# DINT-NSDI24/DINT

Measured on AMD Instinct MI355X. Metric: Mtxn/s + p50/p99 batch latency, TATP, higher is better.
Workload: dtype u64

## Files before the change

### dint_amd/csrc/dint_kv.h

```cpp
#pragma once
#include <cstdlib>
#include <utility>
#include <vector>

#include "dint_kernels.h"
#include "dint_kv_core.h"
#include "state_block.h"
#include "state_image.h"
#include "state_route.h"

#define DINT_KV_MAX_TABLES 5
#define DINT_KV_CTL_BYTES (64 + 24 * KV_NLISTS)
#define DINT_KV_TRACE_WORDS ((size_t)DINT_KV_PMAX * 16 + 16 * 8192)
#define DINT_KV_LOAD_OP 0xF0u

struct kv_dev {
  kv_tab tab[DINT_KV_MAX_TABLES];
  dint_mod mod[DINT_KV_MAX_TABLES];
  dint_mod lockmod[DINT_KV_MAX_TABLES];
  uint32_t gk_base[DINT_KV_MAX_TABLES];
  uint32_t n_tables;
  uint32_t shard_index, shard_count;
  uint32_t same_key;
  uint32_t pass_ins[DINT_KV_MAX_TABLES];
};

struct dint_kv_knobs {
  uint32_t coarse_load = 512;
  uint32_t cap = 0;
  uint32_t lcap = 1024;
  uint32_t cap_mult = 64;
  uint32_t rpt = 0;
  uint32_t no_bm = 0;
  uint32_t hot_min = 0;
  uint32_t no_split = 0;
  uint32_t split_min = 65;
  uint32_t split_target = 384;
  uint32_t one_big_kernel = 0;
  uint32_t workers = 96;
  uint32_t part_first = 0;
  uint32_t sb_split_min = 65;
  uint32_t sb_npmax = 128;
  uint32_t sb_workers = 130;
  uint32_t sb_late_grid = 32;
  uint32_t residency = 0;
  uint32_t no_fuse = 0;
  uint32_t no_ahead = 0;
  uint32_t late_grid = 8;
  uint32_t exp_no_late = 0;
  uint32_t late_fat = 0;
  uint32_t late_big = 0;
};

struct dint_kv {
  uint32_t workload = 0;
  uint32_t n_tables = 0;
  uint32_t val_size = 0;
  int force_rounds = 0;
  uint64_t hash_size[DINT_KV_MAX_TABLES] = {0, 0, 0, 0, 0};
  kv_dev h{};
  kv_dev *d_dev = nullptr;
  uint8_t *d_ctl = nullptr;
  uint64_t *d_trace = nullptr;
  size_t entry_bytes[DINT_KV_MAX_TABLES] = {0, 0, 0, 0, 0};
  dint_kv_knobs knobs;
};

static inline uint32_t dint_kv_cap_mult() {
  const char *v = getenv("DINT_KV_CAP_MULT");
  const unsigned long m = v && *v ? strtoul(v, nullptr, 10) : 64ul;
  return (uint32_t)(m < 2 ? 2 : m > 256 ? 256 : m);
}
static inline uint32_t dint_kv_hash_sizes(uint32_t workload, uint64_t n_rows, uint64_t hs[DINT_KV_MAX_TABLES], uint32_t *val_size) {
  uint32_t n_tables;
  for (uint32_t t = 0; t < DINT_KV_MAX_TABLES; t++) hs[t] = 0;
  if (workload == DINT_WL_STORE) {
    const uint64_t n = n_rows ? n_rows : 2000000ull;
    n_tables = 1;
    *val_size = 40;
    hs[0] = n * 18 / 4;
  } else if (workload == DINT_WL_TATP) {
    const uint64_t n = n_rows ? n_rows : 7000000ull;
    n_tables = 5;
    *val_size = 40;
    hs[0] = hs[1] = n * 3 / 2 / 4;
    hs[2] = hs[3] = n * 15 / 4 / 4;
    hs[4] = n * 45 / 8 / 4;
  } else {
    const uint64_t n = n_rows ? n_rows : 24000000ull;
    n_tables = 2;
    *val_size = 8;
    hs[0] = hs[1] = n * 3 / 2 / 4;
  }
  for (uint32_t t = 0; t < n_tables; t++)
    if (hs[t] == 0) hs[t] = 1;
  return n_tables;
}
int dint_kv_create(dint_kv *kv, uint32_t workload, uint64_t n_rows, dint_shard shard, uint32_t pool_entries = 0,
                   uint32_t flags = 0);
void dint_kv_destroy(dint_kv *kv);
std::vector<std::pair<void *, size_t>> dint_kv_regions(dint_kv *kv);
int64_t dint_kv_dump_rows(dint_kv *kv, uint32_t table, uint64_t *keys, uint32_t *vers, uint8_t *vals, uint64_t cap);
int64_t dint_kv_read_locks(dint_kv *kv, uint32_t table, uint32_t *a, uint32_t *b, uint64_t cap);
struct dint_kv_ahead {
  const void *d_req;
  void *d_rep;
  uint32_t n;
  dint_view view;
};
bool dint_kv_ahead_ok(const dint_kv &kv, int load_mode);
bool dint_kv_one_launch(const dint_kv &kv, int load_mode);
void dint_launch_kv(const void *d_req, void *d_rep, uint32_t n, const dint_kv &kv, dint_log log, dint_scratch s,
                    int load_mode, hipStream_t st, hipEvent_t *ev, const dint_view &view = dint_flat_view(),
                    bool part_done = false, const dint_kv_ahead *next = nullptr);
#define DINT_KV_MULTI_MAX 4u
struct dint_kv_pass {
  const void *d_req;
  void *d_rep;
  uint32_t n;
  const dint_kv *kv;
  dint_log log;
  dint_scratch s;
  dint_view view;
};
void dint_launch_kv_multi(const dint_kv_pass *p, uint32_t n_eng, hipStream_t st, bool part_done = false, const dint_kv_pass *next = nullptr);
bool dint_kv_multi_ahead_ok(const dint_kv &kv);
void dint_launch_home_kv(const void *d_req, uint32_t n, const dint_kv &kv, uint8_t *d_home, hipStream_t st);
struct dint_kv_fmt {
  uint32_t msg, type, table, key, val, ver, val_size;
};
dint_kv_fmt dint_kv_format(uint32_t workload);

struct dint_state_scratch {
  unsigned long long *words;
  uint32_t *blk_cnt;
  uint64_t *blk_off;
  uint32_t nb;
  unsigned long long *digest_part;
};
#define DINT_STATE_DIGEST_GRID 2048u
#define DINT_STATE_WORDS 48u
#define DINT_STATE_DIGEST_AT 16u
uint32_t dint_state_blocks(const dint_kv &kv);
void dint_launch_state_digest(const dint_kv &kv, dint_state_scratch s, hipStream_t st);
void dint_launch_state_diff_count(const dint_kv &a, const dint_kv &b, dint_state_scratch s, hipStream_t st);
void dint_launch_state_diff_write(const dint_kv &a, const dint_kv &b, dint_state_scratch s, void *d_records, uint64_t cap, hipStream_t st);
void dint_launch_state_repair_check(const dint_kv &kv, const void *d_records, uint64_t n, dint_state_scratch s, hipStream_t st);
#define DINT_STATE_HOME_AT 14u
void dint_launch_state_home_check(const dint_kv &kv, const void *d_records, uint64_t n, dint_state_scratch s, hipStream_t st);
void dint_launch_state_repair(const dint_kv &kv, const void *d_records, uint64_t n, uint32_t pend_set, dint_dev_stats *stats,
                              dint_state_scratch s, hipStream_t st);

#define DINT_STATE_STATS_GRID 2048u
#define DINT_STATE_STATS_WORDS 80u
struct dint_stats_scratch {
  unsigned long long *part;
  unsigned long long *out;
};
void dint_launch_state_stats(const dint_kv &kv, dint_stats_scratch s, hipStream_t st);

#define DINT_STATE_VERIFY_GRID 2048u
#define DINT_STATE_VERIFY_WORDS 32u
#define DINT_STATE_VERIFY_PARTS (2u * DINT_STATE_VERIFY_GRID + 1u)
struct dint_verify_scratch {
  uint32_t *owner;
  uint64_t owner_n;
  unsigned long long *part;
  unsigned long long *out;
  uint32_t *leaked;
  uint32_t *blk_cnt;
  uint64_t *blk_off;
  uint64_t blk_n;
  unsigned long long *heads;
};
int dint_verify_alloc(const dint_kv &kv, dint_verify_scratch &s, uint32_t flags);
void dint_verify_free(dint_verify_scratch &s);
void dint_launch_state_verify(const dint_kv &kv, dint_verify_scratch s, uint32_t flags, hipStream_t st, hipEvent_t *ev = nullptr);
int dint_verify_collect(const dint_kv &kv, dint_verify_scratch s, uint32_t flags, hipStream_t st, struct dint_table_verify *out,
                        uint64_t *reclaimed);

struct dint_tables_view;
int dint_view_kv(const dint_tables_view *v, const void *out, uint32_t cap_tables, dint_kv *kv);

// ... 156 lines not shown
```

### dint_amd/csrc/k_kv.hip

```cpp
#include "k_kv_dev.h"

dint_kv_fmt dint_kv_format(uint32_t workload) {
  switch (workload) {
    case DINT_WL_STORE: return {53, 0, 0xFFFFFFFFu, 1, 9, 49, 40};
    case DINT_WL_TATP: return {55, 1, 2, 3, 11, 51, 40};
    default: return {23, 1, 2, 3, 11, 19, 8};
  }
}


static inline uint32_t kv_pick_coarse(uint32_t n, uint32_t load) {
  uint64_t c = ((uint64_t)n + load - 1) / load;
  if (c < 1) c = 1;
  if (c > DINT_KV_CMAX) c = DINT_KV_CMAX;
  return (uint32_t)c;
}
static uint32_t kv_env(const char *name, uint32_t dflt) {
  const char *v = getenv(name);
  return v && *v ? (uint32_t)strtoul(v, nullptr, 10) : dflt;
}
static dint_kv_knobs kv_read_knobs() {
  dint_kv_knobs k;
  k.coarse_load = std::min(8192u, std::max(64u, kv_env("DINT_KV_COARSE_LOAD", KVB_T)));
  k.cap = kv_env("DINT_KV_CAP", 0);
  k.lcap = std::min(KVR_LCAP, kv_env("DINT_KV_LCAP", KVR_LCAP));
  k.cap_mult = dint_kv_cap_mult();
  k.rpt = kv_env("DINT_KV_RPT", 0);
  k.no_bm = kv_env("DINT_KV_NO_BM", 0);
  k.hot_min = kv_env("DINT_KV_HOT_MIN", 0);
  k.no_split = kv_env("DINT_KV_NO_SPLIT", 0);
  k.split_min = std::max(65u, kv_env("DINT_KV_SPLIT_MIN", 65u));
  k.split_target = std::min(448u, std::max(8u, kv_env("DINT_KV_SPLIT_TARGET", 384u)));
  k.one_big_kernel = kv_env("DINT_KV_ONE_BIG_KERNEL", 0);
  k.no_ahead = kv_env("DINT_KV_NO_AHEAD", 0);
  k.no_fuse = kv_env("DINT_KV_NO_FUSE", 0);
  k.sb_split_min = kv_env("DINT_KV_SB_SPLIT_MIN", 65u);
  k.sb_late_grid = std::max(1u, std::min(KVB_GRID, kv_env("DINT_KV_SB_LATE_GRID", 32u)));
  k.sb_npmax = std::max(2u, std::min(KSB_NPMAX, kv_env("DINT_KV_SB_NPMAX", 128u)));
  k.sb_workers = kv_env("DINT_KV_SB_WORKERS", k.sb_npmax + 2u);
  if (k.sb_workers) k.sb_workers = std::max(k.sb_workers, k.sb_npmax + 2u);
  k.workers = std::min(1024u, std::max(KVR_NPMAX + 2u, kv_env("DINT_KV_WORKERS", KVW_GRID)));
  k.part_first = kv_env("DINT_KV_PART_FIRST", 0) & 1u;
  k.late_grid = std::min(KVB_GRID, std::max(1u, kv_env("DINT_KV_LATE_GRID", 8u)));
  k.late_big = kv_env("DINT_KV_LATE_BIG", 0);
  k.exp_no_late = kv_env("DINT_EXP_NO_LATE", 0);
  k.late_fat = kv_env("DINT_KV_LATE_FAT", 0);
  return k;
}

static inline bool kv_uses_hot(const dint_kv &kv, int load_mode) {
  return kv.workload != DINT_WL_SMALLBANK && !(kv.force_rounds & 3) && !load_mode && !kv.knobs.no_split;
}
bool dint_kv_one_launch(const dint_kv &kv, int load_mode) {
  return kv_uses_hot(kv, load_mode) && !kv.knobs.one_big_kernel && !kv.knobs.no_fuse;
}
bool dint_kv_ahead_ok(const dint_kv &kv, int load_mode) {
  if (kv.workload == DINT_WL_SMALLBANK) return !load_mode && !kv.knobs.no_ahead && !kv.knobs.no_fuse;
  return kv_uses_hot(kv, load_mode) && !kv.knobs.one_big_kernel && !kv.knobs.no_ahead;
}

static void kv_fill_pass(kv_pass_args &A, const void *d_req, void *d_rep, uint32_t n, const dint_kv &kv, dint_log log,
                         const dint_scratch &s, int load_mode, const dint_view &view, uint32_t tile) {
  const dint_kv_knobs &K = kv.knobs;
  const uint32_t C = kv_pick_coarse(n, K.coarse_load);
  const uint32_t mean = (n + C - 1) / C;
  uint32_t cap = K.cap_mult * mean + 64;
  cap = std::min(cap, (uint32_t)(s.kbins_slots / C));
  cap = std::max(1u, K.cap ? std::min(cap, K.cap) : cap);
  A.req = (const uint8_t *)d_req; A.rep = (uint8_t *)d_rep; A.n = n;
  A.n_tiles = (n + tile - 1) / tile;
  A.kv = kv.d_dev; A.log = log; A.cut = kv_make_cut(C, n); A.cap = cap;
  A.lcap = K.lcap;
  const uint64_t pn = s.kvs.pass_no;
  A.pno = (uint32_t)(pn & 1u);
  A.bin_cnt = s.kvs.bin_cnt[pn & 1]; A.kbins = s.kvs.kbins[pn & 1]; A.ovl = s.kvs.ovl[pn & 1];
  A.big = s.kvs.ctl[pn % 3]; A.big_z = s.kvs.ctl[(pn + 2) % 3];
  A.blk_pub = s.kvs.pub[pn % 3]; A.blk_pub_z = s.kvs.pub[(pn + 2) % 3];
  A.bigrdy = s.kvs.bigrdy;
  A.ovf = s.ovf; A.ovf2 = s.ovf2; A.stats = s.stats;
  A.bigq = s.bigq;
  A.hotpub = s.hotpub;
  A.lateq = s.lateq;
  A.seq = s.pass_seq ? s.pass_seq : 1u;
  A.inv_n = n > 1 ? (uint32_t)((1ull << 32) / n) : 0xFFFFFFFFu;
  A.load_mode = load_mode;
  A.force_flags = kv.force_rounds | (K.no_bm ? 4 : 0) | (int)(K.hot_min << 8);
  A.split_min = kv_uses_hot(kv, load_mode) ? K.split_min : 0xFFFFFFFFu;
  A.split_target = K.split_target;
  A.np_max = KVR_NPMAX;
  A.sb_pieces = 0;
  A.sbx = s.kvs.sbx;
  if (kv.workload == DINT_WL_SMALLBANK && K.sb_split_min && s.kvs.sbx && !(kv.force_rounds & 3) && !load_mode && !K.no_split) {
    A.split_min = std::max(8u, K.sb_split_min);
    A.np_max = K.sb_npmax;
    A.sb_pieces = 1;
  }
  A.has_log = kv.workload != DINT_WL_STORE;
  A.trace = kv.d_trace;
  A.V = view;
}

extern template int kv_piece_residency<DINT_WL_STORE>(int);
extern template int kv_piece_residency<DINT_WL_TATP>(int);
extern template int kv_piece_residency<DINT_WL_SMALLBANK>(int);
extern template void launch_kv_passes<DINT_WL_STORE>(kv_multi_args &, uint32_t, uint32_t, hipStream_t, hipEvent_t *, const dint_kv_knobs &, bool, const kv_multi_args *, uint32_t);
extern template void launch_kv_passes<DINT_WL_TATP>(kv_multi_args &, uint32_t, uint32_t, hipStream_t, hipEvent_t *, const dint_kv_knobs &, bool, const kv_multi_args *, uint32_t);
extern template void launch_kv_passes<DINT_WL_SMALLBANK>(kv_multi_args &, uint32_t, uint32_t, hipStream_t, hipEvent_t *, const dint_kv_knobs &, bool, const kv_multi_args *, uint32_t);

static inline uint32_t kv_pick_rpt(uint32_t n_total, const dint_kv_knobs &K) {
  if (K.rpt == 1 || K.rpt == 2 || K.rpt == 4) return K.rpt;
  return n_total >= 1024u * 1024u ? 4u : n_total >= 256u * 1024u ? 2u : 1u;
}
static inline uint32_t kv_pick_rpt_ahead(uint32_t n, const dint_kv_knobs &K) {
  if (K.rpt == 4 || (K.rpt == 0 && n >= 256u * 1024u)) return 4u;
  return 2u;
}

static void launch_kv_dispatch(uint32_t workload, kv_multi_args &M, uint32_t n_eng, uint32_t rpt, hipStream_t st, hipEvent_t *ev,
                               const dint_kv_knobs &K, bool part_done = false, const kv_multi_args *next = nullptr, uint32_t next_rpt = 0) {
  switch (workload) {
    case DINT_WL_STORE: launch_kv_passes<DINT_WL_STORE>(M, n_eng, rpt, st, ev, K, part_done, next, next_rpt); break;
    case DINT_WL_TATP: launch_kv_passes<DINT_WL_TATP>(M, n_eng, rpt, st, ev, K, part_done, next, next_rpt); break;
    default: launch_kv_passes<DINT_WL_SMALLBANK>(M, n_eng, rpt, st, ev, K, part_done, next, next_rpt); break;
  }
}

void dint_launch_kv(const void *d_req, void *d_rep, uint32_t n, const dint_kv &kv, dint_log log, dint_scratch s,
                    int load_mode, hipStream_t st, hipEvent_t *ev, const dint_view &view, bool part_done, const dint_kv_ahead *next) {
  if (n == 0) return;
  kv_multi_args M;
  memset(&M, 0, sizeof M);
  const uint32_t rpt = kv_pick_rpt(n, kv.knobs), rpt_a = kv_pick_rpt_ahead(n, kv.knobs);
  kv_fill_pass(M.e[0], d_req, d_rep, n, kv, log, s, load_mode, view, part_done ? KVB_T * rpt_a : KV_TB * rpt);
  kv_multi_args N;
  uint32_t next_rpt = 0;
  if (next && next->n && dint_kv_ahead_ok(kv, load_mode)) {
    dint_scratch sn = s;
    sn.kvs.pass_no = s.kvs.pass_no + 1;
    sn.pass_seq = s.pass_seq + 1 >= 0x3FFFFFFFu ? 1u : s.pass_seq + 1;
    next_rpt = kv_pick_rpt_ahead(next->n, kv.knobs);
    memset(&N, 0, sizeof N);
    kv_fill_pass(N.e[0], next->d_req, next->d_rep, next->n, kv, log, sn, load_mode, next->view, KVB_T * next_rpt);
  } else {
    next = nullptr;
  }
  launch_kv_dispatch(kv.workload, M, 1, rpt, st, ev, kv.knobs, part_done, next ? &N : nullptr, next_rpt);
}

void dint_launch_kv_multi(const dint_kv_pass *p, uint32_t n_eng, hipStream_t st, bool part_done, const dint_kv_pass *next) {
  if (n_eng == 0) return;
  kv_multi_args M, N;
  memset(&M, 0, sizeof M);
  uint32_t n_total = 0;
  for (uint32_t k = 0; k < n_eng; k++) n_total += p[k].n;
  const uint32_t rpt = kv_pick_rpt(n_total, p[0].kv->knobs);
  for (uint32_t k = 0; k < n_eng; k++) kv_fill_pass(M.e[k], p[k].d_req, p[k].d_rep, p[k].n, *p[k].kv, p[k].log, p[k].s, 0, p[k].view, KV_TB * rpt);
  uint32_t next_rpt = 0;
  if (next) {
    uint32_t nmax = 0;
    for (uint32_t k = 0; k < n_eng; k++) nmax = std::max(nmax, next[k].n);
    next_rpt = kv_pick_rpt_ahead(nmax, p[0].kv->knobs);
    memset(&N, 0, sizeof N);
    for (uint32_t k = 0; k < n_eng; k++) {
      dint_scratch sn = next[k].s;
      sn.kvs.pass_no = p[k].s.kvs.pass_no + 1;
      sn.pass_seq = p[k].s.pass_seq + 1 >= 0x3FFFFFFFu ? 1u : p[k].s.pass_seq + 1;
      kv_fill_pass(N.e[k], next[k].d_req, next[k].d_rep, next[k].n, *next[k].kv, next[k].log, sn, 0, next[k].view, KVB_T * next_rpt);
    }
  }
  launch_kv_dispatch(p[0].kv->workload, M, n_eng, rpt, st, nullptr, p[0].kv->knobs, part_done, next ? &N : nullptr, next_rpt);
}
bool dint_kv_multi_ahead_ok(const dint_kv &kv) { return dint_kv_ahead_ok(kv, 0) && !kv.knobs.no_fuse; }

__global__ void __launch_bounds__(256)
k_home_kv(const uint8_t *__restrict__ req, uint32_t n, const kv_dev *__restrict__ kv, dint_kv_fmt f,
          uint8_t *__restrict__ home) {
  const uint32_t i = blockIdx.x * 256u + threadIdx.x;
  if (i >= n) return;
  const uint8_t *m = req + (size_t)i * f.msg;
  const uint32_t table = f.table == 0xFFFFFFFFu ? 0 : m[f.table];
  if (table >= kv->n_tables) { home[i] = 0xFF; return; }
  const uint64_t g = dint_fastmod(dint_hash_key(ld_u64(m + f.key)), kv->mod[table]);
  home[i] = (uint8_t)(g % (kv->shard_count ? kv->shard_count : 1));
}
void dint_launch_home_kv(const void *d_req, uint32_t n, const dint_kv &kv, uint8_t *d_home, hipStream_t st) {
  if (n == 0) return;
  hipLaunchKernelGGL(k_home_kv, dim3((n + 255) / 256), dim3(256), 0, st, (const uint8_t *)d_req, n, kv.d_dev,
                     dint_kv_format(kv.workload), d_home);
}

int dint_kv_create(dint_kv *kv, uint32_t workload, uint64_t n_rows, dint_shard shard, uint32_t pool_entries,
                   uint32_t flags) {
  *kv = dint_kv();
  kv->workload = workload;
  kv->h.same_key = (workload == DINT_WL_TATP && (flags & DINT_FLAG_LOCK_SAME_KEY)) ? 1 : 0;
  uint64_t hs[DINT_KV_MAX_TABLES] = {0, 0, 0, 0, 0};
  kv->n_tables = dint_kv_hash_sizes(workload, n_rows, hs, &kv->val_size);
  const uint32_t stride = kv->val_size == 40 ? 256u : 128u;
  const uint32_t count = shard.count ? shard.count : 1;
  kv->h.n_tables = kv->n_tables;
  kv->h.shard_index = shard.index;
  kv->h.shard_count = count;
  for (uint32_t t = 0; t < DINT_KV_MAX_TABLES; t++) kv->h.pass_ins[t] = 0xFFFFFFFFu;
  if (hipMalloc((void **)&kv->d_ctl, DINT_KV_CTL_BYTES * DINT_KV_MAX_TABLES) != hipSuccess) return DINT_ENOMEM;
  hipMemset(kv->d_ctl, 0, DINT_KV_CTL_BYTES * DINT_KV_MAX_TABLES);
  uint64_t gk = 0;
  for (uint32_t t = 0; t < kv->n_tables; t++) {
    if (hs[t] == 0) hs[t] = 1;
    kv->hash_size[t] = hs[t];
    kv_tab &tb = kv->h.tab[t];
    tb.n_local = (hs[t] + count - 1) / count;
    const uint64_t pool = pool_entries ? pool_entries : tb.n_local / 4 + 4096;
    if (pool > 0xFFFFFFF0ull || gk + tb.n_local > 0xFFFFFFF0ull) return DINT_EINVAL;
    tb.pool_cap = (uint32_t)pool;
    tb.stride = stride;
    tb.val_size = kv->val_size;
    kv->entry_bytes[t] = (size_t)(tb.n_local + tb.pool_cap) * stride;
    if (hipMalloc((void **)&tb.entries, kv->entry_bytes[t]) != hipSuccess) return DINT_ENOMEM;
    if (hipMemset(tb.entries, 0, kv->entry_bytes[t]) != hipSuccess) return DINT_EHIP;
    if (hipMalloc((void **)&tb.pool_next, (size_t)tb.pool_cap * 4) != hipSuccess) return DINT_ENOMEM;
    hipMemset(tb.pool_next, 0, (size_t)tb.pool_cap * 4);
    uint8_t *ctl = kv->d_ctl + DINT_KV_CTL_BYTES * t;
    tb.pool_top = (uint32_t *)ctl;
    tb.free_head = (unsigned long long *)(ctl + 64);
    tb.pend_head = (unsigned long long *)(ctl + 64 + 8 * KV_NLISTS);
// ... 162 lines not shown
```

### dint_amd/csrc/k_kv_dev.h

```cpp
#pragma once
#include <algorithm>
#include <cstddef>
#include <cstdlib>
#include <cstring>
#include <utility>
#include <vector>

#include "../../include/dint_abi.h"
#include "dint_kv.h"
#define KVB_SORT_INLINE
#include "dint_bins.h"

template <int WL> struct Fmt;
template <> struct Fmt<DINT_WL_STORE> {
  static constexpr uint32_t MSG = 53, TYPE = 0, KEY = 1, VAL = 9, VER = 49, VS = 40;
  static constexpr bool HAS_TABLE = false;
  static constexpr uint32_t TABLE = 0;
};
template <> struct Fmt<DINT_WL_TATP> {
  static constexpr uint32_t MSG = 55, TYPE = 1, KEY = 3, VAL = 11, VER = 51, VS = 40;
  static constexpr bool HAS_TABLE = true;
  static constexpr uint32_t TABLE = 2;
};
template <> struct Fmt<DINT_WL_SMALLBANK> {
  static constexpr uint32_t MSG = 23, TYPE = 1, KEY = 3, VAL = 11, VER = 19, VS = 8;
  static constexpr bool HAS_TABLE = true;
  static constexpr uint32_t TABLE = 2;
};

template <int WL>
__device__ static inline uint32_t kv_class(uint32_t type, int load_mode) {
  if (load_mode && type == DINT_KV_LOAD_OP) return 1;
  if (WL == DINT_WL_STORE) return type <= 2 ? 1 : 0;
  if (WL == DINT_WL_TATP) {
    switch (type) {
      case 0: case 1: case 2: case 12: case 13: case 18: case 19: case 22: case 23: return 1;
      case 14: case 24: return 2;
      default: return 0;
    }
  }
  return (type <= 5 || type == 17) ? 1 : (type == 6 ? 2 : 0);
}

__device__ static inline uint32_t kv_pay(uint32_t type, uint32_t q, uint32_t kh) {
  return (type == DINT_KV_LOAD_OP ? 31u : type) | (q << 5) | (kh << 7);
}
__device__ static inline uint32_t pay_type(uint32_t p) { const uint32_t t = p & 31u; return t == 31u ? DINT_KV_LOAD_OP : t; }
__device__ static inline uint32_t pay_q(uint32_t p) { return (p >> 5) & 3u; }
__device__ static inline uint32_t pay_kh(uint32_t p) { return (p >> 7) & 511u; }
__device__ static inline uint32_t kv_table_of(const kv_dev *kv, uint32_t gk) {
  uint32_t t = 0;
  for (uint32_t k = 1; k < kv->n_tables; k++) t += gk >= kv->gk_base[k];
  return t;
}

__device__ static inline uint64_t ld_u64(const uint8_t *p) { uint64_t v; __builtin_memcpy(&v, p, 8); return v; }
__device__ static inline uint32_t ld_u32(const uint8_t *p) { uint32_t v; __builtin_memcpy(&v, p, 4); return v; }
__device__ static inline void st_u32(uint8_t *p, uint32_t v) { __builtin_memcpy(p, &v, 4); }

struct kv_dev_mem {
  __device__ static inline uint32_t fetch_add(uint32_t *p, uint32_t v) { return atomicAdd(p, v); }
  __device__ static inline uint32_t load32(uint32_t *p) { return atomicAdd(p, 0u); }
  __device__ static inline void store32(uint32_t *p, uint32_t v) { atomicExch(p, v); }
  __device__ static inline unsigned long long load64(unsigned long long *p) { return atomicAdd(p, 0ull); }
  __device__ static inline bool cas64(unsigned long long *p, unsigned long long exp, unsigned long long des) {
    return atomicCAS(p, exp, des) == exp;
  }
};

__device__ static inline void kv_dev_pend_set(kv_dev &Skv, uint32_t pno) {
  if (threadIdx.x < DINT_KV_MAX_TABLES && (pno & 1u)) Skv.tab[threadIdx.x].pend_head += KV_NLISTS;
}
#define KV_CTL_INS 32u
static_assert(KV_CTL_INS + DINT_KV_MAX_TABLES <= DINT_KV_CTL_WORDS && KV_CTL_INS * 4 >= 128, "a set of control words is DINT_KV_CTL_WORDS; the counts on a line of their own");
__device__ static inline uint32_t kv_dev_word(const kv_dev *kv, const uint32_t *ctl, uint32_t w) {
  constexpr uint32_t at = (uint32_t)(offsetof(kv_dev, pass_ins) / 4);
  return w >= at && w < at + DINT_KV_MAX_TABLES ? ctl[KV_CTL_INS + w - at] : ((const uint32_t *)kv)[w];
}
__device__ static inline void kv_st_agent(uint64_t *p, uint64_t v) { __hip_atomic_store((unsigned long long *)p, (unsigned long long)v, __ATOMIC_RELAXED, __HIP_MEMORY_SCOPE_AGENT); }
__device__ static inline uint64_t kv_ld_agent(const uint64_t *p) { return __hip_atomic_load((const unsigned long long *)p, __ATOMIC_RELAXED, __HIP_MEMORY_SCOPE_AGENT); }
__device__ static inline void kv_st_agent(uint4 *p, const uint4 &v) {
  kv_st_agent((uint64_t *)p, ((uint64_t)v.y << 32) | v.x);
  kv_st_agent((uint64_t *)p + 1, ((uint64_t)v.w << 32) | v.z);
}
__device__ static inline uint4 kv_ld_agent(const uint4 *p) {
  const uint64_t a = kv_ld_agent((const uint64_t *)p), b = kv_ld_agent((const uint64_t *)p + 1);
  return make_uint4((uint32_t)a, (uint32_t)(a >> 32), (uint32_t)b, (uint32_t)(b >> 32));
}

struct kv_cut { uint32_t P, ibits, magic; };
static inline kv_cut kv_make_cut(uint32_t P, uint32_t n) {
  kv_cut c;
  c.P = P;
  c.ibits = 1;
  while (c.ibits < 32 && (1ull << c.ibits) < n) c.ibits++;
  c.magic = P > 1 ? (uint32_t)((1ull << 32) / P) : 0u;
  return c;
}
__device__ static inline uint32_t kv_cut_div(uint32_t gk, const kv_cut &c, uint32_t *bin) {
  if (c.P <= 1) { *bin = 0; return gk; }
  uint32_t q = __umulhi(gk, c.magic), r = gk - q * c.P;
  if (r >= c.P) { r -= c.P; q++; }
  *bin = r;
  return q;
}
__device__ static inline uint32_t kv_cut_gk(uint32_t gq, uint32_t bin, const kv_cut &c) { return gq * c.P + bin; }
__device__ static inline uint64_t kv_rec(uint32_t gq, uint32_t idx, uint32_t pay, const kv_cut &c) {
  return ((uint64_t)gq << (16 + c.ibits)) | ((uint64_t)idx << 16) | (pay & 0xFFFFu);
}
__device__ static inline uint32_t kv_rec_pay(uint64_t r) { return (uint32_t)r & 0xFFFFu; }
__device__ static inline uint32_t kv_rec_idx(uint64_t r, const kv_cut &c) { return (uint32_t)(r >> 16) & (uint32_t)((1ull << c.ibits) - 1ull); }
__device__ static inline uint64_t kv_sort_key(uint64_t r, const kv_cut &c) {
  const uint32_t pay = kv_rec_pay(r);
  return ((r >> (16 + c.ibits)) << (16 + c.ibits)) | ((uint64_t)((pay >> 7) & 511u) << (7 + c.ibits)) |
         ((uint64_t)kv_rec_idx(r, c) << 7) | (pay & 0x7Fu);
}

struct kv_reqinfo {
  uint32_t type, table, cls;
  uint64_t key;
};
template <int WL>
__device__ static inline kv_reqinfo kv_read_request(const uint8_t *m, bool live, const kv_dev *kv, int load_mode) {
  using F = Fmt<WL>;
  kv_reqinfo r = {0, 0, 0, 0};
  if (live) {
    r.type = m[F::TYPE];
    r.table = F::HAS_TABLE ? m[F::TABLE] : 0;
    r.cls = kv_class<WL>(r.type, load_mode);
    if (r.table >= kv->n_tables) r.cls = 0;
    if (r.cls) r.key = ld_u64(m + F::KEY);
  }
  return r;
}

template <int WL>
__device__ static inline bool kv_insert_op(uint32_t type) {
  return WL == DINT_WL_STORE ? type == 2 : WL == DINT_WL_TATP ? (type == 18 || type == 19) : false;
}

struct kv_pass_args {
  const uint8_t *req;
  uint8_t *rep;
  uint32_t n, n_tiles;
  const kv_dev *kv;
  dint_log log;
  kv_cut cut;
  uint32_t cap;
  uint32_t lcap;
  uint32_t *bin_cnt;
  uint4 *kbins;
  uint32_t *big, *big_z;
  uint32_t *blk_pub, *blk_pub_z;
  uint32_t *bigrdy;
  uint64_t *sbx;
  uint32_t np_max;
  uint32_t sb_pieces;
  uint32_t pno;
  uint4 *ovl;
  uint64_t *ovf;
  uint64_t *ovf2;
  uint4 *bigq;
  unsigned long long *hotpub;
  uint4 *lateq;
  uint32_t split_min;
  uint32_t split_target;
  uint32_t inv_n;
  uint32_t seq;
  dint_dev_stats *stats;
  int load_mode, force_flags;
  uint32_t has_log;
  uint64_t *trace;
  dint_view V;
};
struct kv_multi_args { kv_pass_args e[DINT_KV_MULTI_MAX]; };

__device__ static inline uint64_t u4_key(const uint4 &r) { return ((uint64_t)r.y << 32) | r.x; }
__device__ static inline uint64_t u4_meta(const uint4 &r) { return ((uint64_t)r.w << 32) | r.z; }

template <uint32_t TB, uint32_t... Ks>
__device__ __forceinline__ static void kv_copy_tile(const uint4 *__restrict__ s, uint4 *__restrict__ d, uint32_t nv, uint32_t t,
                                                    std::integer_sequence<uint32_t, Ks...>) {
  const uint4 v[] = {s[min(t + Ks * TB, nv - 1)]...};
  ((d[min(t + Ks * TB, nv - 1)] = v[Ks]), ...);
}

template <int RPT, uint32_t TB = KV_TB>
struct kv_part_lds {
  uint32_t Hc[DINT_KV_CMAX];
  uint32_t Sov[2];
  uint32_t Stile;
  uint32_t Sins[DINT_KV_MAX_TABLES];
  uint32_t Swl[TB / 64 * RPT], Swp[TB / 64];
};
template <int WL, int RPT, uint32_t TB = KV_TB>
__device__ __forceinline__ static void kv_part_body(const kv_pass_args &A, kv_part_lds<RPT, TB> &S, bool first_block) {
  using F = Fmt<WL>;
  constexpr uint32_t T = TB * RPT, NWV = TB / 64;
  auto &Hc = S.Hc; auto &Sov = S.Sov; auto &Stile = S.Stile; auto &Swl = S.Swl; auto &Swp = S.Swp;
  const uint32_t t = threadIdx.x, lane = t & 63, wv = t >> 6;
  const uint32_t n = A.n, C = A.cut.P;
  const kv_dev *__restrict__ kv = A.kv;
  const uint8_t *__restrict__ req = A.req;
  uint8_t *rep = A.rep;
  if (t == 0) { Stile = atomicAdd(&A.big[2], 1u); Sov[0] = 0; }
  if (t < DINT_KV_MAX_TABLES) S.Sins[t] = 0;
  for (uint32_t k = t; k < C; k += TB) Hc[k] = 0;
  __syncthreads();
  const uint32_t tile = Stile;
  kv_reqinfo r[RPT];
  size_t moff[RPT];
  uint64_t lm[RPT];
  uint32_t idx[RPT];
#pragma unroll
  for (int j = 0; j < RPT; j++) {
    idx[j] = tile * T + (uint32_t)j * TB + t;
    bool live;
    moff[j] = dint_view_off(A.V, idx[j] < n ? idx[j] : 0, F::MSG, &live);
    live = live && idx[j] < n;
    r[j] = kv_read_request<WL>(req + moff[j], live, kv, A.load_mode);
    lm[j] = __ballot(r[j].cls == 2);
    if (live && !r[j].cls) atomicAdd(&A.stats->bad_requests, 1ULL);
  }
  if (WL != DINT_WL_STORE) {
    if (lane == 0) {
#pragma unroll
      for (int j = 0; j < RPT; j++) Swl[j * NWV + wv] = (uint32_t)__popcll(lm[j]);
    }
    __syncthreads();
    if (t == 0) {
      uint32_t c = 0;
      for (uint32_t w = 0; w < NWV * RPT; w++) c += Swl[w];
      __hip_atomic_store(&A.blk_pub[tile], 0x80000000u | c, __ATOMIC_RELAXED, __HIP_MEMORY_SCOPE_AGENT);
    }
  }
  if (rep != req) {
    const size_t lo = (size_t)tile * T * F::MSG;
    const size_t hi = min((size_t)n * F::MSG, lo + (size_t)T * F::MSG);
    if ((((uintptr_t)req | (uintptr_t)rep) & 15) == 0) {
      constexpr uint32_t K = (T * F::MSG / 16 + TB - 1) / TB;
      const uint32_t nv = (uint32_t)((hi - lo) / 16);
      const uint4 *s = (const uint4 *)(req + lo);
      uint4 *d = (uint4 *)(rep + lo);
      if (nv) kv_copy_tile<TB>(s, d, nv, t, std::make_integer_sequence<uint32_t, K>());
      for (size_t k = lo + (size_t)nv * 16 + t; k < hi; k += TB) rep[k] = req[k];
    } else {
      for (size_t k = lo + t; k < hi; k += TB) rep[k] = req[k];
    }
  }

  uint32_t coarse[RPT], mypos[RPT];
  uint64_t meta[RPT];
#pragma unroll
  for (int j = 0; j < RPT; j++) {
    coarse[j] = KV_NONE; mypos[j] = 0; meta[j] = 0;
    if (r[j].cls == 1) {
      const uint64_t h = dint_hash_key(r[j].key);
      const uint64_t g = dint_fastmod(h, kv->mod[r[j].table]);
      uint32_t local = (uint32_t)g;
      bool mine = true;
      if (kv->shard_count > 1) {
        mine = (uint32_t)(g % kv->shard_count) == kv->shard_index;
        if (!mine && !A.load_mode) atomicAdd(&A.stats->foreign_requests, 1ULL);
        local = (uint32_t)(g / kv->shard_count);
      }
      if (mine) {
        const uint64_t hs = kv->mod[r[j].table].d, dq = dint_fastmod(h, kv->lockmod[r[j].table]) - g;
        const uint32_t q = dq >= 2 * hs ? (dq >= 3 * hs ? 3u : 2u) : (dq >= hs ? 1u : 0u);
        const uint32_t gq = kv_cut_div(kv->gk_base[r[j].table] + local, A.cut, &coarse[j]);
        meta[j] = kv_rec(gq, idx[j], kv_pay(r[j].type, q, (uint32_t)(h >> 40) & 511u), A.cut);
        mypos[j] = atomicAdd(&Hc[coarse[j]], 1u);
        if (kv_insert_op<WL>(r[j].type)) atomicAdd(&S.Sins[r[j].table], 1u);
      }
    }
  }
  __syncthreads();
  for (uint32_t c = t; c < C; c += TB) {
    const uint32_t cnt = Hc[c];
    if (cnt) Hc[c] = atomicAdd(&A.bin_cnt[c], cnt);
  }
  if (WL != DINT_WL_SMALLBANK && t < DINT_KV_MAX_TABLES && S.Sins[t]) atomicAdd(&A.big[KV_CTL_INS + t], S.Sins[t]);
  __syncthreads();
  uint32_t orank[RPT];
  bool over[RPT];
#pragma unroll
  for (int j = 0; j < RPT; j++) {
    over[j] = false; orank[j] = 0;
    if (coarse[j] != KV_NONE) {
      const uint32_t pos = Hc[coarse[j]] + mypos[j];
      if (pos < A.cap) {
        A.kbins[(size_t)coarse[j] * A.cap + pos] = make_uint4((uint32_t)r[j].key, (uint32_t)(r[j].key >> 32), (uint32_t)meta[j], (uint32_t)(meta[j] >> 32));
      } else {
        over[j] = true;
        orank[j] = atomicAdd(&Sov[0], 1u);
      }
    }
  }
  __syncthreads();
  if (Sov[0]) {
    if (t == 0) Sov[1] = atomicAdd(&A.big[1], Sov[0]);
    __syncthreads();
#pragma unroll
// ... 1809 lines not shown
  const uint32_t t = threadIdx.x & 63u;
  const uint2 bs = Sbig[t];
  uint32_t target = A.split_target;
  if (A.V.seg_cap) {
    uint32_t live = t < A.V.n_seg ? min(A.V.seg_cap, *(const uint32_t *)(A.V.cnt + (size_t)t * A.V.cnt_stride)) : 0u, tot;
    (void)wave_excl_scan_u32(live, &tot);
    if (tot < A.n) target = max(8u, (uint32_t)(((uint64_t)target * max(tot, 1u)) / A.n));
  }
  const uint32_t np0 = (bs.y + target - 1) / target;
  const bool hot = bs.y >= A.split_min && np0 <= A.np_max;
  const uint32_t np = hot ? np0 : 0u;
  const uint32_t nent = bs.y ? (np > 1 ? np + 1 : 1u) : 0u;
  uint32_t tot, at = wave_excl_scan_u32(nent, &tot);
  uint32_t base = 0;
  if (t == 0 && tot) base = atomicAdd(&A.big[3], tot);
  base = (uint32_t)__builtin_amdgcn_readfirstlane((int)base);
  at += base;
  const uint32_t bin = b + A.cut.P * t;
  if (nent && !hot) {
    kv_st_agent(A.bigq + KVQ_W * (size_t)at, make_uint4(bin, bs.x, bs.y, KVQ_SUB));
  } else if (nent) {
    uint64_t hk = L.ckey[t], hr = L.hrec[t];
    if (A.sb_pieces) {
      using F = Fmt<DINT_WL_SMALLBANK>;
      const uint32_t sh_g = 16 + A.cut.ibits;
      uint64_t smp[8];
#pragma unroll
      for (uint32_t j = 0; j < 8; j++) smp[j] = kv_ld_agent(&A.ovf[bs.x + (uint32_t)(((uint64_t)(2 * j + 1) * bs.y) >> 4)]);
      uint32_t best = 0, bj = 0;
#pragma unroll
      for (uint32_t j = 0; j < 8; j++) {
        uint32_t c = 0;
#pragma unroll
        for (uint32_t i = 0; i < 8; i++) c += (smp[i] >> sh_g) == (smp[j] >> sh_g) && pay_q(kv_rec_pay(smp[i])) == pay_q(kv_rec_pay(smp[j]));
        if (c > best) { best = c; bj = j; }
      }
      hr = smp[0];
#pragma unroll
      for (uint32_t j = 1; j < 8; j++) if (j == bj) hr = smp[j];
      const uint32_t hidx = (uint32_t)(hr >> 16) & (uint32_t)((1ull << A.cut.ibits) - 1ull);
      hk = ld_u64(A.rep + dint_view_off(A.V, hidx, F::MSG) + F::KEY);
    }
    for (uint32_t p = 0; p < nent; p++) {
      const uint32_t kind = np == 1 ? KVQ_SOLO : (p < np ? KVQ_PIECE : KVQ_REM);
      uint4 *q = A.bigq + KVQ_W * (size_t)(at + p);
      kv_st_agent(q, make_uint4(bin, bs.x, bs.y, kind | (p << 2) | (np << 10)));
      kv_st_agent(q + 1, make_uint4((uint32_t)hk, (uint32_t)(hk >> 32), at, 0u));
      kv_st_agent(q + 2, make_uint4((uint32_t)hr, (uint32_t)(hr >> 32), 0u, 0u));
    }
  }
  asm volatile("s_waitcnt vmcnt(0)" ::: "memory");
  for (uint32_t p = 0; p < nent; p++)
    if (at + p < DINT_KV_BIGQ_MAX) __hip_atomic_store(&A.bigrdy[at + p], A.seq, __ATOMIC_RELAXED, __HIP_MEMORY_SCOPE_AGENT);
  asm volatile("s_waitcnt vmcnt(0)" ::: "memory");
  if (t == 0) atomicAdd(&A.big[6], 1u);
}

template <int WL, uint32_t NT>
__device__ static inline void kv_coarse_bin(const kv_pass_args &A, const kv_dev *kv, uint32_t coarse, uint8_t *lds_raw,
                                            uint2 *Sbig ,
                                            uint32_t cnt, const uint4 &r0, const uint4 &r1, uint64_t *tr) {
  kvr_lds &L = *(kvr_lds *)lds_raw;
  const uint32_t t = threadIdx.x, lane = t & 63, wave = t >> 6;
  const kv_cut &cut = A.cut;
  const uint32_t C = cut.P, cap = A.cap, sh = 16 + cut.ibits;
  const uint32_t idx_mask = (uint32_t)((1ull << cut.ibits) - 1ull);
  const uint4 *__restrict__ recs = A.kbins + (size_t)coarse * cap;
  if (cnt == 0) {
    if (t == 0) atomicAdd(&A.big[6], 1u);
    return;
  }
  const uint32_t n_in = min(cnt, cap);
  const uint32_t novl = cnt > cap ? A.big[1] : 0u;
  if (t == 0) A.bin_cnt[coarse] = 0;
  auto for_each_record = [&](auto &&f) {
    if (t < n_in) f(r0);
    if (t + NT < n_in) f(r1);
    for (uint32_t k0 = 2 * NT; k0 < n_in; k0 += 8 * NT) {
      uint4 q4[8];
#pragma unroll
      for (uint32_t j = 0; j < 8; j++) {
        const uint32_t k = k0 + j * NT + t;
        q4[j] = k < n_in ? recs[k] : make_uint4(0, 0, 0, 0);
      }
#pragma unroll
      for (uint32_t j = 0; j < 8; j++)
        if (k0 + j * NT + t < n_in) f(q4[j]);
    }
    for (uint32_t k0 = 0; k0 < novl; k0 += 8 * NT) {
      uint32_t b8[8];
#pragma unroll
      for (uint32_t j = 0; j < 8; j++) {
        const uint32_t k = k0 + j * NT + t;
        b8[j] = k < novl ? A.ovl[2 * (size_t)k + 1].x : KV_NONE;
      }
#pragma unroll
      for (uint32_t j = 0; j < 8; j++)
        if (b8[j] == coarse) f(A.ovl[2 * (size_t)(k0 + j * NT + t)]);
    }
  };
  auto big_rec = [&](uint64_t m) -> uint64_t { return ((m >> (sh + 6)) << sh) | (m & ((1ull << sh) - 1ull)); };
  for_each_record([&](const uint4 &r) {
    const uint64_t m = u4_meta(r);
    const uint32_t sub = (uint32_t)(m >> sh) & (KVR_F - 1);
    const uint32_t sub0 = (uint32_t)__builtin_amdgcn_readfirstlane((int)sub);
    const uint64_t same = __ballot(sub == sub0);
    if (sub != sub0) atomicAdd(&L.hist[sub], 1u);
    else if (lane == (uint32_t)__ffsll((unsigned long long)same) - 1) atomicAdd(&L.hist[sub], (uint32_t)__popcll(same));
    if (L.cflag[sub] == 0 && atomicCAS(&L.cflag[sub], 0u, 1u) == 0u) { L.ckey[sub] = u4_key(r); L.hrec[sub] = big_rec(m); }
  });
  __syncthreads();
  if (tr && t == 0) tr[2] = __builtin_amdgcn_s_memrealtime();
  if (wave == 0) {
    const uint32_t h = L.hist[lane];
    bool big = h > 64;
    uint32_t stot, sc = big ? 0u : h, soff = wave_excl_scan_u32(sc, &stot);
    if (stot > A.lcap) {
      big = h > 0; sc = 0; soff = 0; stot = 0;
    }
    uint32_t btot = 0, boff = 0, gbase = 0;
    if (__ballot(big)) {
      boff = wave_excl_scan_u32(big ? h : 0u, &btot);
      if (lane == 0) {
        gbase = atomicAdd(&A.big[0], btot);
        atomicAdd(&A.stats->big_bin_requests, (unsigned long long)btot);
      }
      gbase = (uint32_t)__builtin_amdgcn_readfirstlane((int)gbase);
    }
    L.off[lane] = soff;
    if (lane == 63) L.off[KVR_F] = stot;
    L.bigoff[lane] = big ? gbase + boff : KV_NONE;
    Sbig[lane] = make_uint2(big ? gbase + boff : 0u, big ? h : 0u);
    uint32_t lo = lane + 1, hi = KVR_F;
#pragma unroll
    for (int it = 0; it < 7; it++) {
      const uint32_t mid = min((lo + hi + 1) >> 1, KVR_F);
      const uint32_t v = (uint32_t)__shfl((int)soff, (int)(mid & (KVR_F - 1)), 64);
      const uint32_t om = mid == KVR_F ? stot : v;
      if (lo < hi) {
        if (om - soff <= 64u) lo = mid; else hi = mid - 1;
      }
    }
    uint32_t s = 0, nch = 0;
    while (s < KVR_F) {
      const uint32_t e = (uint32_t)__builtin_amdgcn_readlane((int)lo, (int)s);
      const uint32_t os = (uint32_t)__builtin_amdgcn_readlane((int)soff, (int)s);
      const uint32_t oe = e >= KVR_F ? stot : (uint32_t)__builtin_amdgcn_readlane((int)soff, (int)e);
      if (oe > os) {
        if (lane == 0) L.chs[nch] = make_uint2(os, oe);
        nch++;
      }
      s = e;
    }
    if (lane == 0) L.nch = nch;
    if (tr && lane == 0) { tr[14] = cnt; tr[15] = btot; tr[16] = nch; }
  }
  __syncthreads();
  if (tr && t == 0) tr[3] = __builtin_amdgcn_s_memrealtime();
  for_each_record([&](const uint4 &r) {
    const uint64_t m = u4_meta(r);
    const uint32_t sub = (uint32_t)(m >> sh) & (KVR_F - 1);
    const uint32_t sub0 = (uint32_t)__builtin_amdgcn_readfirstlane((int)sub);
    const uint64_t same = __ballot(sub == sub0);
    const int lead = __ffsll((unsigned long long)same) - 1;
    uint32_t pos = 0;
    if (sub != sub0) pos = atomicAdd(&L.cur[sub], 1u);
    else if ((int)lane == lead) pos = atomicAdd(&L.cur[sub], (uint32_t)__popcll(same));
    if (sub == sub0) pos = (uint32_t)__builtin_amdgcn_readlane((int)pos, lead) + (uint32_t)__popcll(same & lanemask_lt());
    const uint32_t bo = L.bigoff[sub];
    if (bo == KV_NONE) L.rec[L.off[sub] + pos] = r;
    else kv_st_agent(&A.ovf[bo + pos], big_rec(m));
  });
  asm volatile("s_waitcnt vmcnt(0)" ::: "memory");
  __syncthreads();
  if (tr && t == 0) tr[4] = __builtin_amdgcn_s_memrealtime();
  if (wave == NT / 64 - 1) kv_list_items(A, coarse, L, Sbig);
  const uint32_t nch = L.nch;
  for (uint32_t ch = wave; ch < nch; ch += NT / 64) {
    const uint2 ab = L.chs[ch];
    const uint32_t c = ab.y - ab.x;
    const bool has = lane < c;
    const uint4 r = has ? L.rec[ab.x + lane] : make_uint4(0, 0, 0, 0);
    const uint64_t key0 = u4_key(r), m = u4_meta(r);
    const uint32_t pay0 = kv_rec_pay(m);
    uint64_t w = ~0ull;
    if (has) w = ((m >> sh) << (15 + cut.ibits)) | ((uint64_t)pay_kh(pay0) << (6 + cut.ibits)) | ((uint64_t)((uint32_t)(m >> 16) & idx_mask) << 6) | lane;
    w = wave_sort_u64(w);
    uint64_t *ctr = (tr && ch == 0) ? tr + 2 : nullptr;
    if (ctr && lane == 0) tr[5] = __builtin_amdgcn_s_memrealtime();
    const bool valid = lane < c;
    const int src = (int)((uint32_t)w & 63u);
    const uint64_t key = shfl_u64(key0, src);
    const uint32_t pay = (uint32_t)__shfl((int)pay0, src, 64);
    const uint32_t gk = kv_cut_gk((uint32_t)(w >> (15 + cut.ibits)), coarse, cut), kh = (uint32_t)(w >> (6 + cut.ibits)) & 511u;
    const uint32_t idx = (uint32_t)(w >> 6) & idx_mask;
    kv_chunk<WL>(A.rep, valid, valid ? idx : 0, gk, kh, pay_type(pay), valid ? kv_table_of(kv, gk) : 0, pay_q(pay), key, kv, A.stats,
                 A.force_flags & 1, true, A.V, ctr);
  }
}

template <int WL>
__device__ __forceinline__ static void kv_resolve_role(const kv_pass_args &A, uint32_t b, kv_dev &Skv, uint8_t *Lraw, uint2 *Sbig) {
  constexpr uint32_t NT = KVB_T;
  const uint32_t t = threadIdx.x;
  uint64_t *tr = A.trace ? A.trace + 32 * (size_t)b : nullptr;
  if (tr && t == 0) tr[0] = __builtin_amdgcn_s_memrealtime();
  static_assert(sizeof(kv_dev) / 4 <= NT, "one word of the table descriptors per thread");
  const uint4 *__restrict__ recs = A.kbins + (size_t)b * A.cap;
  const uint4 r0 = t < A.cap ? recs[t] : make_uint4(0, 0, 0, 0);
  const uint4 r1 = t + NT < A.cap ? recs[t + NT] : make_uint4(0, 0, 0, 0);
  const uint32_t kvw = t < sizeof(kv_dev) / 4 ? kv_dev_word(A.kv, A.big, t) : 0u;
  const uint32_t cnt = A.bin_cnt[b];
  if (t < sizeof(kv_dev) / 4) ((uint32_t *)&Skv)[t] = kvw;
  if (t < KVR_F) {
    Sbig[t] = make_uint2(0u, 0u);
    kvr_lds &L = *(kvr_lds *)Lraw;
    L.hist[t] = 0; L.cur[t] = 0; L.cflag[t] = 0;
  }
  if (b == 0) {
    if (t < 16 || (t >= KV_CTL_INS && t < KV_CTL_INS + DINT_KV_MAX_TABLES)) A.big_z[t] = 0;
    for (uint32_t k = t; k < 1024; k += NT) A.blk_pub_z[k] = 0;
  }
  __syncthreads();
  kv_dev_pend_set(Skv, A.pno);
  if (tr && t == 0) tr[1] = __builtin_amdgcn_s_memrealtime();
  kv_coarse_bin<WL, NT>(A, &Skv, b, Lraw, Sbig, cnt, r0, r1, tr);
  if (tr && t == 0) { tr[11] = tr[12] = __builtin_amdgcn_s_memrealtime(); tr[13] = b; }
}
template <int WL>
__global__ void __launch_bounds__(KVB_T, 4) k_kv_resolve(kv_multi_args M, uint32_t n_eng) {
  __shared__ kv_dev Skv;
  __shared__ __attribute__((aligned(16))) uint8_t Lraw[sizeof(kvr_lds)];
  __shared__ uint2 Sbig[KVR_F];
  uint32_t e = 0, b = blockIdx.x;
  while (e + 1 < n_eng && b >= M.e[e].cut.P) { b -= M.e[e].cut.P; e++; }
  kv_resolve_role<WL>(M.e[e], b, Skv, Lraw, Sbig);
}

__device__ static inline unsigned long long kvh_word(uint32_t seq, bool ok, uint32_t nwr, int lw_idx, int ll_acq) {
  return ((unsigned long long)(seq & 0x3FFFFFFFu) << 34) | ((unsigned long long)(ok ? 1u : 0u) << 33) | ((unsigned long long)nwr << 23) |
         (lw_idx >= 0 ? (1ull << 22) | ((unsigned long long)(uint32_t)lw_idx << 2) : 0ull) | (ll_acq >= 0 ? 2ull | (unsigned long long)(ll_acq & 1) : 0ull);
}
struct kvh_lds {
  uint32_t key[KVB_T];
  uint32_t idx[KVB_T];
  uint8_t typ[KVB_T];
  uint64_t rem[KVB_T];
  uint64_t all[KVB_T];
  uint16_t cs[KVB_T + 2];
  uint64_t Bw[KVB_W], Bl[KVB_W], Ba[KVB_W];
  unsigned long long pub[KVR_NPMAX + 1];
  uint32_t bad, timeout, nhot, nrem, nall, nsame, nbr, nch, too_big;
  uint32_t found, link, slot, ver0, la0, table;
  uint32_t rowv[10];
  uint32_t best;
  unsigned long long hkey;
  uint32_t ev_ver[KVB_T];
  int16_t ev_src[KVB_T];
  uint8_t ev_ex[KVB_T];
  uint32_t fin_ex, fin_ver, fin_multi, fin_miss, dupf;
  int fin_src;
  uint8_t qq[KVB_T];
  uint64_t Lq[4][KVB_W], Aq[4][KVB_W];
  uint32_t lockw, bestg, gbad;
};
template <int WL>
__device__ __forceinline__ static bool kv_rem_chunks(uint8_t *rep, const kv_cut cut2, const kv_dev *kv, uint32_t bin, uint64_t *R, uint32_t m,
                                                     kvh_lds &H, dint_dev_stats *__restrict__ stats, int force_rounds, const dint_view V,
                                                     bool sorted = false ) {
  using F = Fmt<WL>;
  const uint32_t t = threadIdx.x, lane = t & 63, wave = t >> 6;
  const uint32_t sh_g = 16 + cut2.ibits, sh_k = 7 + cut2.ibits, idx_mask = (uint32_t)((1ull << cut2.ibits) - 1ull);
  __syncthreads();
  if (!sorted) {
    const uint64_t mine = t < m ? kv_sort_key(R[t], cut2) : ~0ull;
    __syncthreads();
    R[t] = mine;
    __syncthreads();
    uint32_t N = 64;
    while (N < m) N <<= 1;
    kvb_sort_blocked<1>(R, N);
  }
  const uint64_t w = R[t];
  const bool head = t < m && (t == 0 || (R[t - 1] >> sh_g) != (w >> sh_g));
  const uint64_t hm = __ballot(head);
  if (lane == 0) H.Bw[wave] = hm;
  __syncthreads();
  if (t == 0) {
    uint32_t nch = 0, start = 0, prev = 0, big = 0;
    for (uint32_t wv = 0; wv < KVB_W; wv++)
      for (uint64_t mm = H.Bw[wv]; mm; mm &= mm - 1) {
        const uint32_t hp = wv * 64 + (uint32_t)__ffsll((unsigned long long)mm) - 1;
        if (hp == 0) continue;
        if (hp - start > 64) { H.cs[nch++] = (uint16_t)start; start = prev; big |= hp - start > 64; }
        prev = hp;
      }
    if (m - start > 64) { H.cs[nch++] = (uint16_t)start; start = prev; big |= m - start > 64; }
    H.cs[nch++] = (uint16_t)start;
    H.cs[nch] = (uint16_t)m;
    H.nch = nch; H.too_big = big;
  }
  __syncthreads();
  if (H.too_big) return false;
  const uint32_t nch = H.nch;
  for (uint32_t ch = wave; ch < nch; ch += KVB_W) {
    const uint32_t a = H.cs[ch], c = H.cs[ch + 1] - a;
    const bool valid = lane < c;
    const uint64_t wv = valid ? R[a + lane] : ~0ull;
    const uint32_t idx = valid ? (uint32_t)(wv >> 7) & idx_mask : 0, gk = kv_cut_gk((uint32_t)(wv >> sh_g), bin, cut2);
    const uint32_t pay = (uint32_t)wv & 0x7Fu;
    const uint64_t key = valid ? ld_u64(rep + dint_view_off(V, idx, F::MSG) + F::KEY) : 0;
    kv_chunk<WL>(rep, valid, idx, gk, (uint32_t)(wv >> sh_k) & 511u, pay_type(pay), valid ? kv_table_of(kv, gk) : 0, pay_q(pay), key, kv, stats,
                 force_rounds, ch + KVB_W >= nch, V);
  }
  __builtin_amdgcn_fence(__ATOMIC_SEQ_CST, "workgroup");
  __syncthreads();
  return true;
}
#define KVG_MAXW 24u
template <int WL>
__device__ __forceinline__ static bool kv_group_phases(uint8_t *rep, const kv_cut cut2, const kv_dev *kv, uint32_t bin, const uint64_t *R, uint32_t Gs,
                                                       uint32_t Ge, kvh_lds &H, dint_dev_stats *__restrict__ stats, const dint_view V) {
  using F = Fmt<WL>;
  const uint32_t t = threadIdx.x, lane = t & 63, wave = t >> 6, n = Ge - Gs;
  const uint32_t sh_g = 16 + cut2.ibits, idx_mask = (uint32_t)((1ull << cut2.ibits) - 1ull);
  auto is_set = [](uint32_t type) -> bool { return WL == DINT_WL_STORE ? type == 1 : (type == 12 || type == 13); };
  auto is_ins = [](uint32_t type) -> bool { return WL == DINT_WL_STORE ? type == 2 : (type == 18 || type == 19); };
  auto is_del = [](uint32_t type) -> bool { return WL == DINT_WL_TATP && (type == 22 || type == 23); };
  const uint32_t gk = kv_cut_gk((uint32_t)(R[Gs] >> sh_g), bin, cut2), table = kv_table_of(kv, gk);
  const kv_tab tb = kv->tab[table];
  const uint64_t bucket = (uint64_t)(gk - kv->gk_base[table]);
  uint8_t *ie = kv_entry_ptr(tb, bucket, KV_INLINE);
  __syncthreads();
  {
    const uint64_t w = t < n ? R[Gs + t] : 0;
    const uint32_t idx = (uint32_t)(w >> 7) & idx_mask, pay = (uint32_t)w & 0x7Fu;
    H.key[t] = t < n ? (idx << 9) | t : 0xFFFFFFFFu;
    H.typ[t] = (uint8_t)(pay_type(pay) & 0xFFu);
    H.qq[t] = (uint8_t)pay_q(pay);
    H.rem[t] = t < n ? ld_u64(rep + dint_view_off(V, idx, F::MSG) + F::KEY) : 0;
    if (t == 0) { H.gbad = 0; H.lockw = KV_LD(uint32_t, ie + KV_LOCKB_OFF); }
  }
  __syncthreads();
  kvb_sort_blocked_u32<1>(H.key, KVB_T);
  const uint32_t sk = H.key[t];
  const bool v = sk != 0xFFFFFFFFu;
  const uint32_t slot = sk & 511u, my_idx = sk >> 9, my_type = v ? H.typ[slot] : 0xFFu, my_q = v ? H.qq[slot] : 0u;
  const uint64_t my_key = v ? H.rem[slot] : 0;
  const bool isW = v && (is_set(my_type) || is_ins(my_type) || is_del(my_type)), isR = v && my_type == 0;
  const bool lk = v && kv_lock_op<WL>(my_type), aq = v && WL == DINT_WL_TATP && my_type == 1;
  if (v && !(kv_simple_op<WL>(my_type) || kv_struct_op<WL>(my_type))) H.gbad = 1;
  if (v && is_ins(my_type) && kv_pool_low(kv, table)) H.gbad = 1;
  const uint64_t bw = __ballot(isW);
  if (lane == 0) H.Bw[wave] = bw;
  if (WL == DINT_WL_TATP) {
#pragma unroll
    for (uint32_t q = 0; q < 4; q++) {
      const uint64_t ml = __ballot(lk && my_q == q), ma = __ballot(aq && my_q == q);
      if (lane == 0) { H.Lq[q][wave] = ml; H.Aq[q][wave] = ma; }
    }
  }
  __syncthreads();
  uint32_t ev_below = 0, nW = 0;
#pragma unroll
  for (uint32_t wv = 0; wv < KVB_W; wv++) {
// ... 1216 lines not shown
```

Measured before the change: 3065.

## Bound speculative bin prefetch and repack sub-bin chunks to cut chunk count

The resolve kernel now preloads bin records speculatively only up to a 'pre' bound, defaulting to the mean bin size plus slack rounded up to 64, instead of the full cap. Records beyond that bound are fetched after the bin count is read. Separately, when the number of per-wave chunks is larger than the 64-record packing minimum, sub-bins are re-placed by a wave-level best-fit pass into fewer chunks, and the offsets are rewritten. The aim is to cut wasted loads and raise lane utilisation during processing. The cost is an extra dependent load for oversized bins and a serial ballot loop for the repacking.

```diff
diff --git a/dint_amd/csrc/dint_kv.h b/dint_amd/csrc/dint_kv.h
--- a/dint_amd/csrc/dint_kv.h
+++ b/dint_amd/csrc/dint_kv.h
@@ -29,6 +29,7 @@
   uint32_t coarse_load = 512;
   uint32_t cap = 0;
   uint32_t lcap = 1024;
+  uint32_t pre = 0;
   uint32_t cap_mult = 64;
   uint32_t rpt = 0;
   uint32_t no_bm = 0;
diff --git a/dint_amd/csrc/k_kv.hip b/dint_amd/csrc/k_kv.hip
--- a/dint_amd/csrc/k_kv.hip
+++ b/dint_amd/csrc/k_kv.hip
@@ -24,6 +24,7 @@
   k.coarse_load = std::min(8192u, std::max(64u, kv_env("DINT_KV_COARSE_LOAD", KVB_T)));
   k.cap = kv_env("DINT_KV_CAP", 0);
   k.lcap = std::min(KVR_LCAP, kv_env("DINT_KV_LCAP", KVR_LCAP));
+  k.pre = kv_env("DINT_KV_PRELOAD", 0);
   k.cap_mult = dint_kv_cap_mult();
   k.rpt = kv_env("DINT_KV_RPT", 0);
   k.no_bm = kv_env("DINT_KV_NO_BM", 0);
@@ -71,6 +72,7 @@
   A.n_tiles = (n + tile - 1) / tile;
   A.kv = kv.d_dev; A.log = log; A.cut = kv_make_cut(C, n); A.cap = cap;
   A.lcap = K.lcap;
+  A.pre = std::min(cap, K.pre ? K.pre : (mean + 64 + 63) / 64 * 64);
   const uint64_t pn = s.kvs.pass_no;
   A.pno = (uint32_t)(pn & 1u);
   A.bin_cnt = s.kvs.bin_cnt[pn & 1]; A.kbins = s.kvs.kbins[pn & 1]; A.ovl = s.kvs.ovl[pn & 1];
diff --git a/dint_amd/csrc/k_kv_dev.h b/dint_amd/csrc/k_kv_dev.h
--- a/dint_amd/csrc/k_kv_dev.h
+++ b/dint_amd/csrc/k_kv_dev.h
@@ -148,6 +148,7 @@
   kv_cut cut;
   uint32_t cap;
   uint32_t lcap;
+  uint32_t pre;
   uint32_t *bin_cnt;
   uint4 *kbins;
   uint32_t *big, *big_z;
@@ -2263,6 +2264,27 @@
       }
       s = e;
     }
+    constexpr uint32_t NW = NT / 64;
+    if ((nch + NW - 1) / NW > ((stot + 63) / 64 + NW - 1) / NW) {
+      uint32_t room = 64, place = 0;
+      for (uint32_t s = 64; s; s--) {
+        for (uint64_t m = __ballot(sc == s); m; m &= m - 1) {
+          const int l = __ffsll((unsigned long long)m) - 1;
+          const int j = __ffsll((unsigned long long)__ballot(room >= s)) - 1;
+          const uint32_t r = (uint32_t)__builtin_amdgcn_readlane((int)room, j);
+          if ((int)lane == j) room = r - s;
+          if ((int)lane == l) place = ((uint32_t)j << 8) | (64u - r);
+        }
+      }
+      const uint32_t used = 64u - room, nch2 = (uint32_t)__popcll(__ballot(used != 0));
+      uint32_t ctot, cbase = wave_excl_scan_u32(used, &ctot);
+      const uint32_t mybase = (uint32_t)__shfl((int)cbase, (int)(place >> 8), 64);
+      if (nch2 < nch) {
+        nch = nch2;
+        L.off[lane] = mybase + (place & 255u);
+        if (lane < nch) L.chs[lane] = make_uint2(cbase, cbase + used);
+      }
+    }
     if (lane == 0) L.nch = nch;
     if (tr && lane == 0) { tr[14] = cnt; tr[15] = btot; tr[16] = nch; }
   }
@@ -2318,10 +2340,14 @@
   if (tr && t == 0) tr[0] = __builtin_amdgcn_s_memrealtime();
   static_assert(sizeof(kv_dev) / 4 <= NT, "one word of the table descriptors per thread");
   const uint4 *__restrict__ recs = A.kbins + (size_t)b * A.cap;
-  const uint4 r0 = t < A.cap ? recs[t] : make_uint4(0, 0, 0, 0);
-  const uint4 r1 = t + NT < A.cap ? recs[t + NT] : make_uint4(0, 0, 0, 0);
+  const uint32_t pre = A.pre;
+  uint4 r0 = t < pre ? recs[t] : make_uint4(0, 0, 0, 0);
+  uint4 r1 = t + NT < pre ? recs[t + NT] : make_uint4(0, 0, 0, 0);
   const uint32_t kvw = t < sizeof(kv_dev) / 4 ? kv_dev_word(A.kv, A.big, t) : 0u;
   const uint32_t cnt = A.bin_cnt[b];
+  const uint32_t n_reg = min(cnt, A.cap);
+  if (t >= pre && t < n_reg) r0 = recs[t];
+  if (t + NT >= pre && t + NT < n_reg) r1 = recs[t + NT];
   if (t < sizeof(kv_dev) / 4) ((uint32_t *)&Skv)[t] = kvw;
   if (t < KVR_F) {
     Sbig[t] = make_uint2(0u, 0u);
```

Result: no change. 3075, median of 6 (+0.3%).
